# tsurumeso/vocal-remover

Hardware: AMD Instinct MI355X
Metric: spectrogram-frames/sec (inference, CascadedNet n_fft=2048) (higher is better)
Workload: dtype f32; 1 GPU; configs[1]: 30 s stereo 44.1 kHz synthetic song, STFT -> 11 crops of 256 frames in one device batch -> predict_mask -> stitch -> mask apply -> iSTFT x2; n_fft=2048, hop=1024, cropsize=256, parallelism=replicas x1 (songs shard, no collective), input_residency=inputs resident in HBM when the timed region starts

## Files before the change

### vocal-remover_amd/csrc/conv_x3h.hip

```cpp
#include <cstdlib>
#include <type_traits>

#include "conv_epilogue.h"
#include "conv_stage.h"
#include "kernels.h"
#include "lds_dma.h"
#include "x3h_common.h"

namespace vr {

template <int MT, int TH, bool UP = true>
struct X3hCfg {
    static constexpr int TW = 32, CK = 8, KK = 9;
    static constexpr int TH_in = TH + 2, PW = TW + 2;
    static constexpr int NSLOT = TH_in * PW;
    static constexpr int NPASS = (NSLOT + 255) / 256;
    static constexpr int WM = MT / 32, WN = TH / 4;
    static constexpr int PLANE = NSLOT * 16;
    static constexpr int P_BYTES = 2 * PLANE;
    static constexpr int NWP = KK * 2 * MT;
    static constexpr int W_BYTES = NWP * 16;
    static constexpr int NWPASS = (NWP + 255) / 256;
    static constexpr int LROWS = TH / 2 + 3, LW = 20, LSLOT = LROWS * LW;
    static constexpr int L_OFF = P_BYTES + 2 * W_BYTES;
    static constexpr int L_BYTES = UP ? CK * LSLOT * 4 : 0;
    static constexpr int E_OFF = L_OFF + L_BYTES;
    static constexpr int M_OFF = E_OFF + 4 * MT * 4;
    static constexpr int LDS_BYTES = M_OFF + 16;
    static constexpr int OCC = (MT == 32 && TH == 8) ? 3 : 2;
    static constexpr int NXL = 8 * NPASS, NWMIN = (NWP / 64) / 4;
    static constexpr int NG = 14;
    static_assert(TH % 4 == 0 && MT % 32 == 0 && LDS_BYTES <= 80 * 1024 && 2 * NXL + NWMIN < 64 && NXL <= 30 && LSLOT <= 256, "tile");
};

__device__ long long g_x3h_trace[4 * 4 * 6 * 8];
void x3h_trace_read(long long* host, int n) {
    VR_HIP(hipMemcpyFromSymbol(host, HIP_SYMBOL(g_x3h_trace), sizeof(long long) * (size_t)(n < 768 ? n : 768)));
}
void x3h_trace_clear() {
    static long long zeros[768] = {0};
    VR_HIP(hipMemcpyToSymbol(HIP_SYMBOL(g_x3h_trace), zeros, sizeof zeros));
}

template <int MT, int TH, bool UP, bool HI, bool TRACE = false>
__global__ __launch_bounds__(256, (X3hCfg<MT, TH>::OCC + (HI ? 1 : 0))) void conv_x3h_kernel(const ConvArgs a) {
    using Cfg = X3hCfg<MT, TH, UP>;
    constexpr int TW = Cfg::TW, KK = Cfg::KK, PW = Cfg::PW, NSLOT = Cfg::NSLOT, NPASS = Cfg::NPASS, WM = Cfg::WM, WN = Cfg::WN,
                  PLANE = Cfg::PLANE, NWP = Cfg::NWP, NWPASS = Cfg::NWPASS;
    extern __shared__ __attribute__((aligned(16))) char smem_x3h[];
    char* const Pb = smem_x3h;

    const int id = blockIdx.x;
    const int xcd = id & 7;
    const int rr = id >> 3;
    const int ct = rr % a.nct;
    const int per_xcd = (a.npt + 7) >> 3;
    const int pt = (a.dbg & 16) ? (rr / a.nct) * 8 + xcd : xcd * per_xcd + rr / a.nct;
    if (pt >= a.npt) return;
    const int tiles_per_img = a.tiles_h * a.tiles_w;
    const int n = pt / tiles_per_img;
    const int trem = pt - n * tiles_per_img;
    const int h0 = (trem / a.tiles_w) * TH;
    const int w0 = (a.wt0 + trem % a.tiles_w) * TW;
    const int co0 = ct * MT;
    const int tid = threadIdx.x;
    const int lane = tid & 63;
    const int wave = __builtin_amdgcn_readfirstlane(tid >> 6);
    const int nchunk = (a.Cin + 7) >> 3;
    const unsigned lds0 = (unsigned)(size_t)smem_x3h;
    const int dbg = a.dbg & 15;
    const bool prio = (a.dbg & 32) != 0;
    const int trace_wg = TRACE ? (int)blockIdx.x - (int)(gridDim.x / 2) : -1;
    auto stamp = [&](int k, int point) {
        if (TRACE && trace_wg >= 0 && trace_wg < 4 && k >= 2 && k < 8) {
            const long long t = __builtin_readcyclecounter();
            if (lane == 0) g_x3h_trace[((trace_wg * 4 + wave) * 6 + (k - 2)) * 8 + point] = t;
        }
    };

    auto pixel_offset = [&](int p, unsigned sH4) -> int {
        const int s = p * 256 + tid;
        const int r = s / PW, c = s - r * PW;
        const int hi = h0 - 1 + r, wi = w0 - 1 + c;
        const bool ok = s < NSLOT && hi >= 0 && hi < a.Hin && wi >= 0 && wi < a.Win;
        return ok ? (int)((unsigned)hi * sH4 + (unsigned)(wi * 4)) : (int)0x80000000u;
    };
    const ConvSrc& us = a.src[0].up ? a.src[0] : (a.src[1].up ? a.src[1] : a.src[2]);
    constexpr bool any_up = UP;
    int lrow = 0, lcol4 = 0;
    int lidx[NPASS], lstep[NPASS];
    float lh[NPASS], lw_[NPASS];
// ... 8 lines not shown
            const int s = p * 256 + tid;
            const int r = s / PW, c = s - r * PW;
            const int hi = h0 - 1 + r, wi = w0 - 1 + c;
            const bool ok = s < NSLOT && hi >= 0 && hi < a.Hin && wi >= 0 && wi < a.Win;
            const float h1r = us.rh * (float)(ok ? hi : 0), w1r = us.rw * (float)(ok ? wi : 0);
            const int h1 = (int)h1r, w1 = (int)w1r;
            lidx[p] = ok ? ((h1 - lr0) * Cfg::LW + (w1 - lc0)) * 32 : -1;
            const int rs = (h1 + 1 < us.H && h1 + 1 - lr0 < Cfg::LROWS) ? Cfg::LW * 32 : 0;
            const int cs = (w1 + 1 < us.W && w1 + 1 - lc0 < Cfg::LW) ? 32 : 0;
            lstep[p] = (rs << 16) | cs;
            lh[p] = h1r - (float)h1;
            lw_[p] = w1r - (float)w1;
        }
    }
    unsigned woff0;
    {
        const int q = wave * 64 + lane;
        const int m = q % MT, tp = q / MT;
        woff0 = (unsigned)((tp * a.CoutPad + m) * 16);
    }
    const unsigned wstep = (unsigned)((256 / MT) * a.CoutPad * 16);
    const long long wchunk_bytes = (long long)KK * 2 * a.CoutPad * 16;
    auto issue_w = [&](int k) {
        const char* wb = static_cast<const char*>(a.x3w) + k * wchunk_bytes + (long long)co0 * 16;
        const i32x4 wr = make_rsrc(reinterpret_cast<const float*>(wb), (unsigned)(wchunk_bytes - (long long)co0 * 16));
        const unsigned ws_b = lds0 + (unsigned)(Cfg::P_BYTES + (k & 1) * Cfg::W_BYTES);
#pragma unroll
        for (int i = 0; i < NWPASS; ++i) {
            const int pp = wave + 4 * i;
            if ((pp + 1) * 64 <= NWP) dma16s(ws_b + pp * 1024, woff0, wr, (unsigned)i * wstep);
            else if (pp * 64 + lane < NWP) dma16s(ws_b + pp * 1024, woff0, wr, (unsigned)i * wstep);
        }
    };
    const float* xp = a.src[0].p + (long long)n * a.src[0].sN;
    long long xsC = a.src[0].sC;
    unsigned xsH4 = (unsigned)a.src[0].sH * 4u;
    int xend = a.c1, xsi = 0;
    bool xup = a.src[0].up != 0;
    unsigned upm[2] = {0u, 0u};
    int xvo[NPASS];
#pragma unroll
    for (int p = 0; p < NPASS; ++p) xvo[p] = pixel_offset(p, xsH4);
    auto next_source = [&]() {
        ++xsi;
        if (xsi == 1) { xp = a.src[1].p + (long long)n * a.src[1].sN; xsC = a.src[1].sC; xsH4 = (unsigned)a.src[1].sH * 4u; xend = a.c2; xup = a.src[1].up != 0; }
        else { xp = a.src[2].p + (long long)n * a.src[2].sN; xsC = a.src[2].sC; xsH4 = (unsigned)a.src[2].sH * 4u; xend = 1 << 30; xup = a.src[2].up != 0; }
#pragma unroll
        for (int p = 0; p < NPASS; ++p) xvo[p] = pixel_offset(p, xsH4);
    };
    float xr[2][NPASS][8];
    auto load_channel = [&](int k, int cl, auto par) {
        constexpr int PAR = decltype(par)::value;
        const int ci = k * 8 + cl;
        const bool live = ci < a.Cin && dbg != 1;
        if (live && ci >= xend) next_source();
        if (live && ci >= xend) next_source();
        const i32x4 xs = make_rsrc(xp, live ? 0x7FFFFFF0u : 0u);
        const bool up = UP && live && xup;
        if (cl == 0) upm[PAR] = 0u;
        upm[PAR] |= (up ? 1u : 0u) << cl;
        xr[PAR][0][cl] = x3h_load(xs, up ? (int)((unsigned)lrow * xsH4) + lcol4 : xvo[0]);
        const i32x4 xs1 = make_rsrc(xp, (live && !up) ? 0x7FFFFFF0u : 0u);
#pragma unroll
        for (int p = 1; p < NPASS; ++p) xr[PAR][p][cl] = x3h_load(xs1, xvo[p]);
        if (live) xp += xsC;
    };
    auto wait_pixels = [&](auto par, auto newer) {
        constexpr int PAR = decltype(par)::value, NEWER = decltype(newer)::value;
#pragma unroll
        for (int p = 0; p < NPASS; ++p) x3h_wait8<NEWER>(xr[PAR][p]);
    };
    auto stage_lowres = [&](auto par) {
        constexpr int PAR = decltype(par)::value;
        if (upm[PAR] == 0u) return;
        if (tid < Cfg::LSLOT) {
            vr_f32x4h lo4, hi4;
// ... 79 lines not shown
    };

    const int khalf = lane >> 5, l31 = lane & 31;
    const int bq = (wave * WN * PW + l31) * 16;
    const int bX = bq + khalf * PLANE, bY1 = bq + khalf * 16, bY2 = bq + khalf * (PW - 2) * 16;
    const int aX = l31 * 16, aY = (MT + l31 + khalf * 2 * MT) * 16;

    f32x16 acc[WM][WN];
#pragma unroll
    for (int mi = 0; mi < WM; ++mi)
#pragma unroll
        for (int ni = 0; ni < WN; ++ni)
#pragma unroll
            for (int r = 0; r < 16; ++r) acc[mi][ni][r] = 0.f;

    using P0 = std::integral_constant<int, 0>;
    using P1 = std::integral_constant<int, 1>;
    float ecv[4];
    {
        const int ec = co0 + (tid & (MT - 1));
        const int ecc = ec < a.Cout ? ec : a.Cout - 1;
        const i32x4 rb = make_rsrc(a.bias, a.bias ? 0x7FFFFFF0u : 0u);
        const i32x4 re = make_rsrc(a.epi, a.epi ? 0x7FFFFFF0u : 0u);
        const i32x4 rw = make_rsrc(reinterpret_cast<const float*>(static_cast<const char*>(a.x3w) + nchunk * wchunk_bytes), 0x7FFFFFF0u);
        ecv[0] = x3h_load(rb, ecc * 4);
        ecv[1] = x3h_load(re, ecc * 8);
        ecv[2] = x3h_load(re, ecc * 8 + 4);
        ecv[3] = x3h_load(rw, ec * 4);
    }
    auto follow = [&](int e, bool first) {
        const int need = 140 - (e < 14 ? 14 : e);
        shlo = (first || need < shlo) ? need : shlo;
        int nsh = sh;
        if (first || need < sh - 1) nsh = need;
        else if (need > sh + 12) {
            nsh = need < sh + 64 ? need : sh + 64;
            nsh = nsh < shlo + 64 ? nsh : shlo + 64;
            nsh = nsh > sh ? nsh : sh;
        }
        if (nsh != sh) {
            if (!first) {
                const int d = nsh - sh;
                const float f = d < -126 ? 0.f : x3h_pow2(d);
#pragma unroll
                for (int mi = 0; mi < WM; ++mi)
#pragma unroll
                    for (int ni = 0; ni < WN; ++ni)
#pragma unroll
                        for (int r = 0; r < 16; ++r) acc[mi][ni][r] *= f;
            }
            sh = nsh;
            psc = x3h_pow2(sh);
        }
    };
#pragma unroll
    for (int cl = 0; cl < 8; ++cl) load_channel(0, cl, P0{});
    issue_w(0);
#pragma unroll
    for (int cl = 0; cl < 8; ++cl) load_channel(1, cl, P1{});
    wait_pixels(P0{}, std::integral_constant<int, Cfg::NXL + Cfg::NWMIN>{});
    asm volatile("; landed %0 %1 %2 %3" : "+v"(ecv[0]), "+v"(ecv[1]), "+v"(ecv[2]), "+v"(ecv[3]));
    if (tid < MT) {
        float* E = reinterpret_cast<float*>(smem_x3h + Cfg::E_OFF);
        E[tid] = ecv[0];
        E[MT + tid] = a.epi ? ecv[1] : 1.f;
        E[2 * MT + tid] = a.epi ? ecv[2] : 0.f;
        E[3 * MT + tid] = ecv[3];
    }
    post_max(P0{});
    if (any_up) stage_lowres(P0{});
    lds_barrier();
    follow(read_max_exp(), true);
    convert(P0{});
    asm volatile("s_waitcnt vmcnt(%0) lgkmcnt(0)" :: "n"(Cfg::NXL) : "memory");
    __builtin_amdgcn_s_barrier();
    asm volatile("" ::: "memory");

    auto chunk = [&](int k, auto par) {
        constexpr int PAR = decltype(par)::value;
        const bool more = k + 1 < nchunk;
        stamp(k, 0);
        {
            const char* Wb = smem_x3h + Cfg::P_BYTES + PAR * Cfg::W_BYTES;
            vr_f16x8 A[2][WM], B[2][WN];
            auto read_group = [&](int g, int buf) {
                const bool isY = g == 13 || (g < 12 && g % 3 == 2);
                const int t = g >= 12 ? 8 : 2 * (g / 3) + (g % 3 == 1 ? 1 : 0);
                const int ty = t / 3, tx = t % 3;
#pragma unroll
                for (int mi = 0; mi < WM; ++mi) {
                    const char* q = Wb + (t * 2 * MT + mi * 32) * 16;
                    if (!isY) A[buf][mi] = *reinterpret_cast<const vr_f16x8*>(q + aX);
                    else if (t < 8) A[buf][mi] = *reinterpret_cast<const vr_f16x8*>(q + aY);
                    else {
                        const vr_i32x4 v = *reinterpret_cast<const vr_i32x4*>(q + aX + MT * 16);
                        vr_i32x4 z;
#pragma unroll
                        for (int j = 0; j < 4; ++j) z[j] = khalf ? 0 : v[j];
                        A[buf][mi] = __builtin_bit_cast(vr_f16x8, z);
// ... 18 lines not shown
            if (prio) __builtin_amdgcn_s_setprio(1);
#pragma unroll
            for (int g = 0; g < Cfg::NG; ++g) {
                const int cur = g & 1;
                if (g + 1 < Cfg::NG) read_group(g + 1, cur ^ 1);
                if (more) {
                    if (g == 0) issue_w(k + 1);
                    if (g >= 1 && g <= 4) { load_channel(k + 2, 2 * g - 2, par); load_channel(k + 2, 2 * g - 1, par); }
                }
                __builtin_amdgcn_sched_barrier(0);
                mfma_group(cur);
                __builtin_amdgcn_sched_barrier(0);
            }
            if (prio) __builtin_amdgcn_s_setprio(0);
        }
        stamp(k, 1);
        if (more) {
            using Q = std::integral_constant<int, PAR ^ 1>;
            wait_pixels(Q{}, std::integral_constant<int, Cfg::NXL + Cfg::NWMIN>{});
            stamp(k, 2);
            post_max(Q{});
            if (any_up) stage_lowres(Q{});
            stamp(k, 3);
            lds_barrier();
            stamp(k, 4);
            follow(read_max_exp(), false);
            if (dbg != 3) convert(Q{});
            stamp(k, 5);
            asm volatile("s_waitcnt vmcnt(%0) lgkmcnt(0)" :: "n"(Cfg::NXL) : "memory");
            stamp(k, 6);
            __builtin_amdgcn_s_barrier();
            asm volatile("" ::: "memory");
            stamp(k, 7);
        }
    };
    for (int k = 0; k < nchunk; k += 2) {
        chunk(k, P0{});
        if (k + 1 < nchunk) chunk(k + 1, P1{});
    }
    asm volatile("s_waitcnt vmcnt(0)" ::: "memory");

    if (dbg == 4) return;
    {
        const float fo = x3h_pow2(-sh);
        const float* Wi = reinterpret_cast<const float*>(smem_x3h + Cfg::E_OFF) + 3 * MT;
#pragma unroll
        for (int mi = 0; mi < WM; ++mi)
#pragma unroll
            for (int rq = 0; rq < 4; ++rq) {
                const vr_f32x4h wi = *reinterpret_cast<const vr_f32x4h*>(Wi + mi * 32 + 8 * rq + 4 * khalf);
#pragma unroll
                for (int ni = 0; ni < WN; ++ni)
#pragma unroll
                    for (int j = 0; j < 4; ++j) acc[mi][ni][rq * 4 + j] = (acc[mi][ni][rq * 4 + j] * fo) * wi[j];
            }
    }
    {
        int hon[WN], won[WN];
#pragma unroll
        for (int ni = 0; ni < WN; ++ni) { hon[ni] = h0 + wave * WN + ni; won[ni] = w0 + l31; }
        epi_store<MT, WM, WN>(VR_EPI_ARGS(a), acc, reinterpret_cast<const float*>(smem_x3h + Cfg::E_OFF), n, co0, khalf,
                              h0 + TH <= a.Hout && w0 + TW <= a.Wout, hon, won);
    }
    if (a.part) {
        __syncthreads();
        float* red = reinterpret_cast<float*>(smem_x3h);
#pragma unroll
        for (int mi = 0; mi < WM; ++mi) {
#pragma unroll
            for (int r = 0; r < 16; ++r) {
                float s1 = 0.f, s2 = 0.f;
#pragma unroll
                for (int ni = 0; ni < WN; ++ni) {
                    const int ho = h0 + wave * WN + ni, wo = w0 + l31;
                    if (ho < a.Hout && wo < a.Wout) {
                        const float v = acc[mi][ni][r];
                        s1 += v;
                        s2 = fmaf(v, v, s2);
                    }
                }
                s1 = half_wave_sum_dpp(s1);
                s2 = half_wave_sum_dpp(s2);
                if (l31 == 16) {
                    const int m = mi * 32 + (r & 3) + 8 * (r >> 2) + 4 * khalf;
                    red[(wave * MT + m) * 2 + 0] = s1;
                    red[(wave * MT + m) * 2 + 1] = s2;
                }
// ... 60 lines not shown
}
__global__ void x3h_wscale_batched_kernel(const X3WDesc* __restrict__ d) {
    const X3WDesc e = d[blockIdx.y];
    x3h_wscale_block(e.w, e.o, e.Cin, e.KK, e.CoutPad, blockIdx.x);
}
__global__ void x3h_weights_batched_kernel(const X3WDesc* __restrict__ d) {
    const X3WDesc e = d[blockIdx.y];
    x3h_weights_elem(e.w, e.o, e.Cin, e.KK, e.CoutPad, (long long)blockIdx.x * blockDim.x + threadIdx.x);
}

void launch_x3h_weights(const float* w, void* o, int Cin, int KK, int CoutPad, hipStream_t st) {
    const long long n = (long long)((Cin + 7) / 8 * 8) * KK * CoutPad;
    VR_LAUNCH(x3h_wscale_kernel, dim3((unsigned)((CoutPad + 31) / 32)), dim3(256), 0, st, w, o, Cin, KK, CoutPad);
    VR_LAUNCH(x3h_weights_kernel, dim3((unsigned)((n + 255) / 256)), dim3(256), 0, st, w, o, Cin, KK, CoutPad);
    VR_HIP(hipGetLastError());
}
void launch_x3h_weights_batched(const X3WDesc* d_descs, int n, long long max_elems, int max_cout_pad, hipStream_t st) {
    if (n <= 0) return;
    VR_LAUNCH(x3h_wscale_batched_kernel, dim3((unsigned)((max_cout_pad + 31) / 32), (unsigned)n), dim3(256), 0, st, d_descs);
    VR_LAUNCH(x3h_weights_batched_kernel, dim3((unsigned)((max_elems + 255) / 256), (unsigned)n), dim3(256), 0, st, d_descs);
    VR_HIP(hipGetLastError());
}

template <int MT, int TH, bool UP, bool HI, bool TRACE = false>
static void x3h_launch_up(const ConvArgs& a, hipStream_t st) {
    using Cfg = X3hCfg<MT, TH, UP>;
    auto kern = conv_x3h_kernel<MT, TH, UP, HI, TRACE>;
    static std::atomic<unsigned long long> attr_done{0};
    ensure_lds_attr(attr_done, reinterpret_cast<const void*>(kern), Cfg::LDS_BYTES);
    const int groups = (a.npt + 7) / 8;
    VR_LAUNCH(kern, dim3(groups * 8 * a.nct), dim3(256), Cfg::LDS_BYTES, st, a);
    VR_HIP(hipGetLastError());
}

template <int MT, int TH>
static void x3h_launch(const ConvArgs& a, hipStream_t st) {
    static const int hi = [] { const char* e = getenv("VR_X3H_HI"); return e ? atoi(e) : 0; }();
    if (a.dbg & 64) {
        if (a.src[0].up | a.src[1].up | a.src[2].up) x3h_launch_up<MT, TH, true, false, true>(a, st);
        else x3h_launch_up<MT, TH, false, false, true>(a, st);
        return;
    }
    if (a.src[0].up | a.src[1].up | a.src[2].up) x3h_launch_up<MT, TH, true, false>(a, st);
    else if (hi && TH == 8) x3h_launch_up<MT, TH, false, (TH == 8)>(a, st);
    else x3h_launch_up<MT, TH, false, false>(a, st);
}

void x3h_launch_conv(const ConvArgs& a, const X3Tile& t, hipStream_t st) {
    if (t.MT == 64) x3h_launch<64, 8>(a, st);
    else if (t.TH == 16) x3h_launch<32, 16>(a, st);
    else x3h_launch<32, 8>(a, st);
}

}
```

### vocal-remover_amd/csrc/model.h

```cpp
#pragma once
#include <chrono>
#include <deque>
#include <functional>
#include <map>
#include <memory>
#include <string>
#include <vector>

#include "kernels.h"

namespace vr {

struct Arena {
    char* base = nullptr;
    size_t cap = 0, off = 0, peak = 0;
    bool dry = false;
    void* alloc(size_t bytes) {
        const size_t a = (off + 255) & ~size_t(255);
        off = a + bytes;
        if (off > peak) peak = off;
        if (dry) return reinterpret_cast<void*>(uintptr_t(256));
        if (off > cap) throw Error(-4, "workspace arena overflow (planning bug)");
        return base + a;
    }
// ... 166 lines not shown
    bool band_fork_active = false;
    bool gs_clear_pending = false;
    bool wgrad_on_side = false;
    struct Lane { hipStream_t main = nullptr, side = nullptr; hipEvent_t fork = nullptr, join = nullptr, start = nullptr, done = nullptr; Arena ws; };
    std::vector<Lane> lanes;
    void swap_lane(int i);

private:
    float* p_arena = nullptr; size_t p_floats = 0;
    float* b_arena = nullptr; size_t b_floats = 0;
    Arena ws;
    Arena io;
    void ensure_ws(size_t bytes);
    int plan_B = -1, plan_T = -1; bool plan_training = false; size_t plan_peak = 0;
    void ensure_io(size_t bytes);

    std::deque<BN> bns;
    std::vector<BN*> bn_list;
    std::vector<Conv*> wino_list;
    struct PendingConv { ConvArgs a; ConvShape shp; double flops, bytes; bool stats; BNFinalizeArgs fin; BN* bn; };
    std::vector<PendingConv>* conv_sink = nullptr;
    int x3d_mode = 2;
    int conv_w_lo = 0, conv_w_hi = 0;
    std::vector<Conv*> x3d_list;
    float* wino_arena = nullptr;
    float* winot_arena = nullptr;
    std::map<const Param*, float*> winot_of;
    char* wino6_arena = nullptr;
    char* winot6_arena = nullptr;
    std::map<const Param*, void*> winot6_of;
    char* x3_arena = nullptr;
    char* x3t_arena = nullptr;
    std::map<const Param*, void*> x3t_of;
    std::map<const Param*, void*> x3dt_of;
    std::vector<WgReduceDesc> wred_host, wred_sent;
    WgReduceDesc* wred_dev = nullptr;
    size_t wred_cap = 0;
    void flush_wgrad_sums();
    struct X3Batch { std::vector<X3WDesc> host; X3WDesc* dev = nullptr; long long max_elems = 0; };
    X3Batch xb_fwd, xb_bwd;
    void run_x3_batch(X3Batch& b, std::vector<X3WDesc>& descs);
    void refresh_wino(bool with_dgrad);
    struct WinoBatch { std::vector<WinoWDesc> host; WinoWDesc* dev = nullptr; long long max_elems = 0; };
    WinoBatch wb_fwd, wb_bwd, wb_fwd6, wb_bwd6;
    void run_wino_batch(WinoBatch& b, std::vector<WinoWDesc>& descs, bool split6);
    BNFoldDesc* d_fold = nullptr;
// ... 119 lines not shown
```

### vocal-remover_amd/csrc/model.hip

```cpp
#include "model.h"

#include <algorithm>
#include <chrono>
#include <cmath>
#include <cstdlib>
#include <cstring>

namespace vr {

static inline int round_up(int v, int m) { return (v + m - 1) / m * m; }

Param* Model::add_param(const std::string& key, std::vector<int64_t> shape, ParamKind kind, bool trainable) {
    params.emplace_back();
    Param* p = &params.back();
    p->key = key;
    p->shape = std::move(shape);
    p->kind = kind;
    p->trainable = trainable;
    p->numel = 1;
    for (auto d : p->shape) p->numel *= (size_t)d;
    p->dev_numel = p->numel;
    if (kind == PK_CONV) {
        p->Cout = (int)p->shape[0];
        p->Cin = (int)p->shape[1];
// ... 77 lines not shown
    ihr->Cout = 4 * hid; ihr->Cin = nin_lstm; ihr->KK = 1; ihr->CoutPad = M.proj.CoutPad; ihr->co_off = 4 * hid;
    ihr->dev_numel = 0; ihr->alias_of = ihf;
    M.proj.w = ihf;
    M.dense.name = q + ".dense";
    M.dense.Cin = 2 * hid; M.dense.Cout = nin_lstm; M.dense.CoutPad = round_up(nin_lstm, 32);
    M.dense.KS = 1; M.dense.stride = 1; M.dense.pad_h = M.dense.pad_w = 0; M.dense.slope = 0.f;
    M.dense.w = add_param(q + ".dense.0.weight", {nin_lstm, 2 * hid}, PK_CONV, true);
    M.dense_b = add_param(q + ".dense.0.bias", {nin_lstm}, PK_PLAIN, true);
    M.dense.bn = add_bn(q + ".dense.1", nin_lstm, 0);
    build_cba(B.dec[3], p + ".dec1.conv1", 3 * c + 1, c, 3, 1, 1, 1, 1, 1, RELU);
}

Model::Model(int device_, int n_fft_, int hop_, int nout_, int nout_lstm_, bool is_complex_)
    : device(device_), n_fft(n_fft_), hop(hop_), nout(nout_), nout_lstm(nout_lstm_), is_complex(is_complex_), nin(is_complex_ ? 4 : 2) {
    VR_CHECK(n_fft >= 64 && (n_fft & (n_fft - 1)) == 0 && n_fft <= 8192, -2, "n_fft must be a power of two in [64, 8192]");
    VR_CHECK(hop > 0, -2, "hop_length must be positive");
    VR_CHECK(nout % 4 == 0 && nout >= 4 && nout_lstm % 4 == 0 && nout_lstm >= 4, -2, "nout / nout_lstm must be multiples of 4");
    max_bin = n_fft / 2;
    output_bin = n_fft / 2 + 1;
    VR_CHECK((max_bin / 2) % 16 == 0, -2, "n_fft/4 must be a multiple of 16 (four stride-2 encoders)");
    DeviceGuard dev_guard(device);
    if (const char* e = getenv("VR_MFMA_MODE")) { mfma_mode = atoi(e); VR_CHECK(mfma_mode >= 0 && mfma_mode <= 3, -2, "VR_MFMA_MODE: 0, 1, 2 or 3"); }
    default_mfma_mode = mfma_mode;
    VR_HIP(hipStreamCreateWithFlags(&stream, hipStreamNonBlocking));
    if (!getenv("VR_NO_SIDE_STREAM")) {
        VR_HIP(hipStreamCreateWithFlags(&side_stream, hipStreamNonBlocking));
        VR_HIP(hipEventCreateWithFlags(&ev_fork, hipEventDisableTiming));
        VR_HIP(hipEventCreateWithFlags(&ev_join, hipEventDisableTiming));
        if (!getenv("VR_NO_SPLIT_BATCH")) {
            int k = getenv("VR_LANES") ? atoi(getenv("VR_LANES")) : 2;
            k = k < 1 ? 1 : (k > 4 ? 4 : k);
            lanes.resize(k - 1);
            for (Lane& l : lanes) {
                VR_HIP(hipStreamCreateWithFlags(&l.main, hipStreamNonBlocking));
                VR_HIP(hipStreamCreateWithFlags(&l.side, hipStreamNonBlocking));
                VR_HIP(hipEventCreateWithFlags(&l.fork, hipEventDisableTiming));
                VR_HIP(hipEventCreateWithFlags(&l.join, hipEventDisableTiming));
                VR_HIP(hipEventCreateWithFlags(&l.start, hipEventDisableTiming));
                VR_HIP(hipEventCreateWithFlags(&l.done, hipEventDisableTiming));
            }
        }
    }
    const int nin_lstm = max_bin / 2;
    build_basenet(nets_[0], "stg1_low_band_net.0", nin, nout / 2, nin_lstm / 2, nout_lstm);
    build_cba(tail1, "stg1_low_band_net.1", nout / 2, nout / 4, 1, 1, 0, 0, 1, 1, 0.f);
    build_basenet(nets_[1], "stg1_high_band_net", nin, nout / 4, nin_lstm / 2, nout_lstm / 2);
// ... 186 lines not shown
        const int G = 4 * M.hid;
        if (!M.bias_sum) VR_HIP(hipMalloc(reinterpret_cast<void**>(&M.bias_sum), (size_t)2 * G * sizeof(float)));
        launch_add(M.b_ih_f->dev, M.b_hh_f->dev, M.bias_sum, G, stream);
        launch_add(M.b_ih_r->dev, M.b_hh_r->dev, M.bias_sum + G, G, stream);
    }
    affine_dirty = false;
}

void Model::set_option(const std::string& name, int value) {
    plan_peak = 0;
    if (name == "train_winograd") train_wino = value != 0;
    else if (name == "serial_exec") serial = value != 0;
    else if (name == "params_dirty") affine_dirty = true;
    else if (name == "mfma_bf16") { mfma_mode = value != 0 ? 1 : default_mfma_mode; affine_dirty = true; }
    else if (name == "mfma_mode") {
        if (value < -1 || value > 3) throw Error(-2, "mfma_mode: 0, 1, 2, 3 or -1 (default)");
        mfma_mode = value < 0 ? default_mfma_mode : value; affine_dirty = true;
    }
    else if (name == "conv_x3d") {
        if (value < -1 || value > 2) throw Error(-2, "conv_x3d: 0, 1, 2 or -1 (default)");
        x3d_mode = value < 0 ? 2 : value;
    }
    else if (name == "crop_window") crop_window = value != 0;
    else if (name == "adam_reset") reset_adam_state();
    else if (name == "hip_graph" || name == "conv_x3p" || name == "wgrad_x3h" || name == "conv_x3b") {
        static std::string told;
        if (told.find("|" + name + "|") == std::string::npos) {
            told += "|" + name + "|";
            fprintf(stderr, "libvr_mi355: option '%s' was retired with its kernel (tools/experiments/README.md); ignored\n", name.c_str());
        }
    }
    else throw Error(-2, "unknown option: " + name);
}

void Model::refresh_wino(bool with_dgrad) {
    if (!wino_arena) {
        size_t total = 0;
        for (Conv* L : wino_list) total += (size_t)L->Cin * 16 * L->CoutPad;
        VR_HIP(hipMalloc(reinterpret_cast<void**>(&wino_arena), total * sizeof(float)));
        size_t off = 0;
        for (Conv* L : wino_list) { L->wino = wino_arena + off; off += (size_t)L->Cin * 16 * L->CoutPad; }
    }
    {
        std::vector<WinoWDesc> d;
        for (Conv* L : wino_list) d.push_back(WinoWDesc{L->w->dev, L->wino, L->Cin, L->CoutPad});
        run_wino_batch(wb_fwd, d, false);
// ... 349 lines not shown
            if (!x3_pick(probe, ConvShape{L.KS, L.stride, L.dh, L.dw}, &xt)) {
                for (SrcSpec& sp : srcs) {
                    if (!sp.up) continue;
                    const Tensor& t = sp.t;
                    Tensor u;
                    u.N = t.N; u.C = t.C; u.H = 2 * t.H; u.W = 2 * t.W;
                    u.sH = u.W; u.sC = (long long)u.H * u.W; u.sN = u.sC * u.C; u.slope = 1.f;
                    u.p = ws.allocf((size_t)u.N * u.C * u.H * u.W);
                    if (!dry) launch_upsample2x(t, u.p, stream);
                    sp = SrcSpec{u};
                }
                build_fwd_args(L, srcs, N, batch_as_h, a);
            }
        }
    }
    a.bias = bias;
    const bool fuse_epi = !training && L.bn != nullptr;
    if (fuse_epi) { a.epi = L.bn->affine; a.epi_slope = L.slope; }
    a.wino = (training && !train_wino) ? nullptr : L.wino;
    a.wino6 = (a.wino && mfma_mode == 2) ? L.wino6 : nullptr;
    a.x3w = (x3_mode() && !(training && !train_wino)) ? L.x3w : nullptr;
    if (!x3d_mode && a.Win == 16) a.x3w = nullptr;
    a.bf16 = mfma_mode;
    int wcols = a.Wout;
    if (conv_w_hi > 0 && !training && mfma_mode == 3 && !batch_as_h && !conv_sink) {
        X3Tile xt;
        int tth;
        const ConvShape cs{L.KS, L.stride, L.dh, L.dw};
        if (!thin16_pick(a, cs, &tth) && x3_pick(a, cs, &xt)) {
            a.w_lo = conv_w_lo; a.w_hi = conv_w_hi;
            wcols = std::min(a.Wout, (conv_w_hi + 31) / 32 * 32) - conv_w_lo / 32 * 32;
        }
    }
    Tensor o;
    if (batch_as_h) {
        o.N = N; o.C = L.Cout; o.H = 1; o.W = a.Wout;
        if (out_view) { o.p = out_view->p; o.g = out_view->g; o.sN = out_view->sN; o.sC = out_view->sC; o.sH = out_view->sH; }
        else {
            o.p = ws.allocf((size_t)N * L.Cout * a.Wout); o.sN = (long long)L.Cout * a.Wout; o.sC = a.Wout; o.sH = a.Wout;
            if (taping()) o.g = galloc((size_t)N * L.Cout * a.Wout, false);
        }
        a.dst[0] = ConvDst{o.p, 0, o.sC, o.sN, 0};
    } else {
        o.N = N; o.C = L.Cout; o.H = a.Hout; o.W = a.Wout;
        if (out_view) {
            VR_CHECK(out_view->H == a.Hout && out_view->W == a.Wout && out_view->C == L.Cout, -2, "conv " + L.name + ": output view shape mismatch");
// ... 1483 lines not shown
        for (Part& p : parts) {
            VR_CHECK(p.o.out_off == p.need, -4, "stream schedule mismatch (planning bug)");
            if (!out_on_dev && p.need > 0) {
                VR_HIP(hipMemcpy2DAsync(y[p.k], (size_t)capacity[p.k] * 4, p.stage_y, (size_t)p.need * 4, (size_t)p.need * 4, 2, hipMemcpyDeviceToHost, stream));
                VR_HIP(hipMemcpy2DAsync(v[p.k], (size_t)capacity[p.k] * 4, p.stage_v, (size_t)p.need * 4, (size_t)p.need * 4, 2, hipMemcpyDeviceToHost, stream));
            }
        }
        VR_HIP(hipStreamSynchronize(stream));
    } catch (...) {
        hipStreamSynchronize(stream);
        throw;
    }
    for (Part& p : parts) {
        p.S->broken = false;
        if (n_out) n_out[p.k] = p.need;
    }
}

void Model::debug_conv(const float* x, int N, int Cin, int H, int W, const float* w_oihw, int Cout, int KS, int stride,
                       int dh, int dw, int flags, const float* aff, float slope, const float* bias, float* out,
                       float* stats_out) {
    DeviceGuard dev_guard(device);
    const int up = flags & 1;
    const bool want_wino = (flags & 2) != 0, epi = (flags & 4) != 0;
    const int KK = KS * KS, CoutPad = round_up(Cout, 32);
    const int Hin = up ? 2 * H : H, Win = up ? 2 * W : W;
    const int pad_h = KS == 1 ? 0 : dh, pad_w = KS == 1 ? 0 : dw;
    const int Hout = (Hin + 2 * pad_h - dh * (KS - 1) - 1) / stride + 1;
    const int Wout = (Win + 2 * pad_w - dw * (KS - 1) - 1) / stride + 1;
    std::vector<float> wk((size_t)Cin * KK * CoutPad, 0.f);
    for (int co = 0; co < Cout; ++co)
        for (int ci = 0; ci < Cin; ++ci)
            for (int k = 0; k < KK; ++k) wk[((size_t)ci * KK + k) * CoutPad + co] = w_oihw[((size_t)co * Cin + ci) * KK + k];
    float *dx, *dw_, *dout, *daff = nullptr, *dbias = nullptr, *dpart = nullptr;
    const size_t xin = (size_t)N * Cin * H * W, xout = (size_t)N * Cout * Hout * Wout;
    VR_HIP(hipMalloc(&dx, xin * 4)); VR_HIP(hipMalloc(&dw_, wk.size() * 4)); VR_HIP(hipMalloc(&dout, xout * 4));
    VR_HIP(hipMemcpy(dx, x, xin * 4, hipMemcpyHostToDevice));
    VR_HIP(hipMemcpy(dw_, wk.data(), wk.size() * 4, hipMemcpyHostToDevice));
    const size_t naff = epi ? Cout : Cin;
    if (aff) { VR_HIP(hipMalloc(&daff, naff * 8)); VR_HIP(hipMemcpy(daff, aff, naff * 8, hipMemcpyHostToDevice)); }
    if (bias) { VR_HIP(hipMalloc(&dbias, (size_t)Cout * 4)); VR_HIP(hipMemcpy(dbias, bias, (size_t)Cout * 4, hipMemcpyHostToDevice)); }
    Tensor t;
    t.p = dx; t.N = N; t.C = Cin; t.H = H; t.W = W; t.sH = W; t.sC = (long long)H * W; t.sN = t.sC * Cin;
    if (!epi) { t.aff0 = daff; t.slope = slope; }
    ConvArgs a{};
    a.nsrc = 1; a.src[0] = make_src(t, up != 0, 0); a.c1 = a.c2 = Cin; a.Cin = Cin;
    a.w = dw_; a.bias = dbias; a.Cout = Cout; a.CoutPad = CoutPad;
    if (epi && daff) { a.epi = daff; a.epi_slope = slope; }
    a.bf16 = mfma_mode;
    float* dwino = nullptr;
    void* dwino6 = nullptr;
    void* dx3w = nullptr;
    if (want_wino && mfma_mode == 3 && stride == 1 && (KS == 1 || dh > 1)) {
        VR_HIP(hipMalloc(&dx3w, x3_weights_bytes(Cin, KK, CoutPad)));
        launch_x3h_weights(dw_, dx3w, Cin, KK, CoutPad, stream);
        a.x3w = dx3w;
    } else if (want_wino) {
        VR_CHECK(KS == 3 && stride == 1 && dh == 1 && dw == 1, -2, "Winograd weights exist for 3x3 stride-1 convs only");
        VR_HIP(hipMalloc(&dwino, (size_t)Cin * 16 * CoutPad * 4));
        launch_wino_weights(dw_, dwino, Cin, CoutPad, stream);
        a.wino = dwino;
        if (mfma_mode == 2) {
            VR_HIP(hipMalloc(&dwino6, wino_weights6_bytes(Cin, CoutPad)));
            launch_wino_weights6(dw_, dwino6, Cin, CoutPad, stream);
            a.wino6 = dwino6;
            VR_HIP(hipMalloc(&dx3w, x3_weights_bytes(Cin, 9, CoutPad)));
            launch_x3_weights(dw_, dx3w, Cin, 9, CoutPad, stream);
            a.x3w = dx3w;
        }
// ... 2 lines not shown
            launch_x3h_weights(dw_, dx3w, Cin, 9, CoutPad, stream);
            a.x3w = dx3w;
        }
    }
    if (!x3d_mode && Win == 16) a.x3w = nullptr;
    a.dst[0] = ConvDst{dout, (long long)Hout * Wout * Cout, (long long)Hout * Wout, (long long)Wout, 0};
    a.d1 = a.d2 = 1 << 30;
    a.N = N; a.Hout = Hout; a.Wout = Wout; a.Hin = Hin; a.Win = Win; a.pad_h = pad_h; a.pad_w = pad_w;
    const ConvShape shp{KS, stride, dh, dw};
    size_t npt = 0;
    if (stats_out) { npt = conv_part_count(a, shp); VR_HIP(hipMalloc(&dpart, npt * Cout * 8)); a.part = dpart; }
    launch_conv(a, shp, stream);
    VR_HIP(hipStreamSynchronize(stream));
    VR_HIP(hipMemcpy(out, dout, xout * 4, hipMemcpyDeviceToHost));
    if (stats_out) {
        std::vector<float> part(npt * Cout * 2);
        VR_HIP(hipMemcpy(part.data(), dpart, part.size() * 4, hipMemcpyDeviceToHost));
        for (int c = 0; c < Cout; ++c) {
            double s1 = 0, s2 = 0;
            for (size_t i = 0; i < npt; ++i) { s1 += part[(i * Cout + c) * 2]; s2 += part[(i * Cout + c) * 2 + 1]; }
            stats_out[2 * c] = (float)s1; stats_out[2 * c + 1] = (float)s2;
        }
    }
    hipFree(dx); hipFree(dw_); hipFree(dout); hipFree(daff); hipFree(dbias); hipFree(dpart); hipFree(dwino); hipFree(dwino6); hipFree(dx3w);
}

}
```

### vocal-remover_amd/csrc/vr_common.h

```cpp
#pragma once
#include <hip/hip_runtime.h>
#include <atomic>
#include <cstdint>
#include <cstdio>
#include <stdexcept>
#include <string>
#include <vector>

namespace vr {

struct Error : std::runtime_error {
    int code;
    Error(int c, const std::string& m) : std::runtime_error(m), code(c) {}
};

#define VR_HIP(expr)                                                                              \
    do {                                                                                          \
        hipError_t _e = (expr);                                                                   \
        if (_e != hipSuccess)                                                                     \
            throw ::vr::Error(-3, std::string(#expr) + ": " + hipGetErrorString(_e));             \
    } while (0)

#define VR_CHECK(cond, code, msg)                                                                 \
    do {                                                                                          \
// ... 81 lines not shown
    int nsrc, c1, c2;
    int Cin;
    const float* w;
    const float* wino;
    const void* wino6;
    const void* x3w;
    const float* bias;
    int Cout, CoutPad;
    ConvDst dst[3];
    int d1, d2;
    float* part;
    const float* epi;
    float epi_slope;
    int N, Hout, Wout, Hin, Win;
    int pad_h, pad_w;
    int tiles_w, tiles_h, npt, nct;
    int dbg;
    int bf16;
    long long s2_cls_stride;
    int s2_H, s2_W;
    int tapmask;
    int w_lo, w_hi;
    int wt0;
};

struct ConvShape {
    int KS, stride, dil_h, dil_w;
};

struct WgradArgs {
    ConvArgs in;
    const float* dz;
    long long zN, zC, zH;
    int Cout, CoutPad;
    float* part;
    long long part_stride;
    int P, tiles_w, tiles_h, npt, nchunks, nct;
    int dma;
    int bf16;
    int allow_wino;
};
double launch_wgrad(const WgradArgs& a, const ConvShape& s, float* grad_out, int accumulate, hipStream_t st);
struct WgReduceDesc { const float* part; long long stride; float* out; long long n; int P; int accumulate; long long blk0; };
void wgrad_defer_to(std::vector<WgReduceDesc>* sink);
int wgrad_reduce_vec(const WgReduceDesc* host_descs, int n);
void launch_wgrad_reduce_batched(const WgReduceDesc* d_descs, int n, long long total_blocks, int vec, hipStream_t st);
// ... 9 lines not shown
```

Baseline: 173,900 spectrogram-frames/sec.

## Split input-channel reduction across two wave groups in 3x3 conv kernel

Adds a K-split variant of the 32x8 x3h conv kernel. It launches 512 threads, and two 256-thread groups each take alternate 8-channel chunks. The groups sync through an LDS atomic spin barrier, align their shared exponent scale, and reduce partial accumulators through LDS before one group runs the epilogue. The variant is picked during inference when there are many channel chunks but fewer than roughly one workgroup per CU, so that small-grid layers can use more waves. The cost is double the LDS per workgroup, the spin-barrier overhead and an extra reduction pass.

```diff
diff --git a/vocal-remover_amd/csrc/conv_x3h.hip b/vocal-remover_amd/csrc/conv_x3h.hip
--- a/vocal-remover_amd/csrc/conv_x3h.hip
+++ b/vocal-remover_amd/csrc/conv_x3h.hip
@@ -28,6 +28,8 @@
     static constexpr int M_OFF = E_OFF + 4 * MT * 4;
     static constexpr int LDS_BYTES = M_OFF + 16;
     static constexpr int OCC = (MT == 32 && TH == 8) ? 3 : 2;
+    static constexpr int KS_STRIDE = LDS_BYTES + 16;
+    static constexpr int KS_LDS_BYTES = 2 * KS_STRIDE;
     static constexpr int NXL = 8 * NPASS, NWMIN = (NWP / 64) / 4;
     static constexpr int NG = 14;
     static_assert(TH % 4 == 0 && MT % 32 == 0 && LDS_BYTES <= 80 * 1024 && 2 * NXL + NWMIN < 64 && NXL <= 30 && LSLOT <= 256, "tile");
@@ -42,12 +44,26 @@
     VR_HIP(hipMemcpyToSymbol(HIP_SYMBOL(g_x3h_trace), zeros, sizeof zeros));
 }
 
-template <int MT, int TH, bool UP, bool HI, bool TRACE = false>
-__global__ __launch_bounds__(256, (X3hCfg<MT, TH>::OCC + (HI ? 1 : 0))) void conv_x3h_kernel(const ConvArgs a) {
+__device__ __forceinline__ void x3h_group_barrier(int* cnt, int target, int lane) {
+    asm volatile("" ::: "memory");
+    if (lane == 0) __hip_atomic_fetch_add(cnt, 1, __ATOMIC_RELAXED, __HIP_MEMORY_SCOPE_WORKGROUP);
+    for (int spin = 0; spin < (1 << 22); ++spin) {
+        const int v = __builtin_amdgcn_readfirstlane(__hip_atomic_load(cnt, __ATOMIC_RELAXED, __HIP_MEMORY_SCOPE_WORKGROUP));
+        if (v >= target) break;
+        __builtin_amdgcn_s_sleep(1);
+    }
+    asm volatile("" ::: "memory");
+}
+
+template <int MT, int TH, bool UP, bool HI, bool TRACE = false, bool KS = false>
+__global__ __launch_bounds__(KS ? 512 : 256, (X3hCfg<MT, TH>::OCC + (HI ? 1 : 0))) void conv_x3h_kernel(const ConvArgs a) {
     using Cfg = X3hCfg<MT, TH, UP>;
+    static_assert(!KS || (MT == 32 && TH == 8 && !UP && HI && !TRACE), "the K-split form exists for the plain 32 x 8 tiling only");
     constexpr int TW = Cfg::TW, KK = Cfg::KK, PW = Cfg::PW, NSLOT = Cfg::NSLOT, NPASS = Cfg::NPASS, WM = Cfg::WM, WN = Cfg::WN,
                   PLANE = Cfg::PLANE, NWP = Cfg::NWP, NWPASS = Cfg::NWPASS;
-    extern __shared__ __attribute__((aligned(16))) char smem_x3h[];
+    extern __shared__ __attribute__((aligned(16))) char smem_x3h_wg[];
+    const int grp = KS ? __builtin_amdgcn_readfirstlane((int)threadIdx.x >> 8) : 0;
+    char* const smem_x3h = smem_x3h_wg + (KS ? grp * Cfg::KS_STRIDE : 0);
     char* const Pb = smem_x3h;
 
     const int id = blockIdx.x;
@@ -63,10 +79,12 @@
     const int h0 = (trem / a.tiles_w) * TH;
     const int w0 = (a.wt0 + trem % a.tiles_w) * TW;
     const int co0 = ct * MT;
-    const int tid = threadIdx.x;
+    const int tid = KS ? (int)(threadIdx.x & 255) : (int)threadIdx.x;
     const int lane = tid & 63;
     const int wave = __builtin_amdgcn_readfirstlane(tid >> 6);
-    const int nchunk = (a.Cin + 7) >> 3;
+    const int nchunk_all = (a.Cin + 7) >> 3;
+    const int nchunk = KS ? (nchunk_all - grp + 1) >> 1 : nchunk_all;
+    auto gch = [&](int j) -> int { return KS ? 2 * j + grp : j; };
     const unsigned lds0 = (unsigned)(size_t)smem_x3h;
     const int dbg = a.dbg & 15;
     const bool prio = (a.dbg & 32) != 0;
@@ -121,7 +139,7 @@
     const unsigned wstep = (unsigned)((256 / MT) * a.CoutPad * 16);
     const long long wchunk_bytes = (long long)KK * 2 * a.CoutPad * 16;
     auto issue_w = [&](int k) {
-        const char* wb = static_cast<const char*>(a.x3w) + k * wchunk_bytes + (long long)co0 * 16;
+        const char* wb = static_cast<const char*>(a.x3w) + gch(k) * wchunk_bytes + (long long)co0 * 16;
         const i32x4 wr = make_rsrc(reinterpret_cast<const float*>(wb), (unsigned)(wchunk_bytes - (long long)co0 * 16));
         const unsigned ws_b = lds0 + (unsigned)(Cfg::P_BYTES + (k & 1) * Cfg::W_BYTES);
 #pragma unroll
@@ -150,7 +168,19 @@
     float xr[2][NPASS][8];
     auto load_channel = [&](int k, int cl, auto par) {
         constexpr int PAR = decltype(par)::value;
-        const int ci = k * 8 + cl;
+        const int ci = gch(k) * 8 + cl;
+        if constexpr (KS) {
+            if (cl == 0 && gch(k) > 0) {
+#pragma unroll
+                for (int c = 0; c < 8; ++c) {
+                    const int cs = ci - 8 + c;
+                    const bool lv = cs < a.Cin && dbg != 1;
+                    if (lv && cs >= xend) next_source();
+                    if (lv && cs >= xend) next_source();
+                    if (lv) xp += xsC;
+                }
+            }
+        }
         const bool live = ci < a.Cin && dbg != 1;
         if (live && ci >= xend) next_source();
         if (live && ci >= xend) next_source();
@@ -276,7 +306,7 @@
         const int ecc = ec < a.Cout ? ec : a.Cout - 1;
         const i32x4 rb = make_rsrc(a.bias, a.bias ? 0x7FFFFFF0u : 0u);
         const i32x4 re = make_rsrc(a.epi, a.epi ? 0x7FFFFFF0u : 0u);
-        const i32x4 rw = make_rsrc(reinterpret_cast<const float*>(static_cast<const char*>(a.x3w) + nchunk * wchunk_bytes), 0x7FFFFFF0u);
+        const i32x4 rw = make_rsrc(reinterpret_cast<const float*>(static_cast<const char*>(a.x3w) + nchunk_all * wchunk_bytes), 0x7FFFFFF0u);
         ecv[0] = x3h_load(rb, ecc * 4);
         ecv[1] = x3h_load(re, ecc * 8);
         ecv[2] = x3h_load(re, ecc * 8 + 4);
@@ -307,28 +337,44 @@
             psc = x3h_pow2(sh);
         }
     };
-#pragma unroll
-    for (int cl = 0; cl < 8; ++cl) load_channel(0, cl, P0{});
-    issue_w(0);
-#pragma unroll
-    for (int cl = 0; cl < 8; ++cl) load_channel(1, cl, P1{});
-    wait_pixels(P0{}, std::integral_constant<int, Cfg::NXL + Cfg::NWMIN>{});
-    asm volatile("; landed %0 %1 %2 %3" : "+v"(ecv[0]), "+v"(ecv[1]), "+v"(ecv[2]), "+v"(ecv[3]));
-    if (tid < MT) {
-        float* E = reinterpret_cast<float*>(smem_x3h + Cfg::E_OFF);
-        E[tid] = ecv[0];
-        E[MT + tid] = a.epi ? ecv[1] : 1.f;
-        E[2 * MT + tid] = a.epi ? ecv[2] : 0.f;
-        E[3 * MT + tid] = ecv[3];
-    }
-    post_max(P0{});
-    if (any_up) stage_lowres(P0{});
-    lds_barrier();
-    follow(read_max_exp(), true);
-    convert(P0{});
-    asm volatile("s_waitcnt vmcnt(%0) lgkmcnt(0)" :: "n"(Cfg::NXL) : "memory");
-    __builtin_amdgcn_s_barrier();
-    asm volatile("" ::: "memory");
+    int* const gcnt = reinterpret_cast<int*>(smem_x3h + Cfg::LDS_BYTES);
+    int gbar = 0;
+    auto sync_waves = [&]() {
+        if constexpr (KS) { gbar += 4; x3h_group_barrier(gcnt, gbar, lane); }
+        else __builtin_amdgcn_s_barrier();
+    };
+    auto sync_lds = [&]() {
+        if constexpr (KS) { asm volatile("s_waitcnt lgkmcnt(0)" ::: "memory"); sync_waves(); }
+        else lds_barrier();
+    };
+    if constexpr (KS) {
+        if (tid == 0) *gcnt = 0;
+        lds_barrier();
+    }
+    if (!KS || nchunk > 0) {
+#pragma unroll
+        for (int cl = 0; cl < 8; ++cl) load_channel(0, cl, P0{});
+        issue_w(0);
+#pragma unroll
+        for (int cl = 0; cl < 8; ++cl) load_channel(1, cl, P1{});
+        wait_pixels(P0{}, std::integral_constant<int, Cfg::NXL + Cfg::NWMIN>{});
+        asm volatile("; landed %0 %1 %2 %3" : "+v"(ecv[0]), "+v"(ecv[1]), "+v"(ecv[2]), "+v"(ecv[3]));
+        if (tid < MT) {
+            float* E = reinterpret_cast<float*>(smem_x3h + Cfg::E_OFF);
+            E[tid] = ecv[0];
+            E[MT + tid] = a.epi ? ecv[1] : 1.f;
+            E[2 * MT + tid] = a.epi ? ecv[2] : 0.f;
+            E[3 * MT + tid] = ecv[3];
+        }
+        post_max(P0{});
+        if (any_up) stage_lowres(P0{});
+        sync_lds();
+        follow(read_max_exp(), true);
+        convert(P0{});
+        asm volatile("s_waitcnt vmcnt(%0) lgkmcnt(0)" :: "n"(Cfg::NXL) : "memory");
+        sync_waves();
+        asm volatile("" ::: "memory");
+    }
 
     auto chunk = [&](int k, auto par) {
         constexpr int PAR = decltype(par)::value;
@@ -393,14 +439,14 @@
             post_max(Q{});
             if (any_up) stage_lowres(Q{});
             stamp(k, 3);
-            lds_barrier();
+            sync_lds();
             stamp(k, 4);
             follow(read_max_exp(), false);
             if (dbg != 3) convert(Q{});
             stamp(k, 5);
             asm volatile("s_waitcnt vmcnt(%0) lgkmcnt(0)" :: "n"(Cfg::NXL) : "memory");
             stamp(k, 6);
-            __builtin_amdgcn_s_barrier();
+            sync_waves();
             asm volatile("" ::: "memory");
             stamp(k, 7);
         }
@@ -411,6 +457,47 @@
     }
     asm volatile("s_waitcnt vmcnt(0)" ::: "memory");
 
+    if constexpr (KS) {
+        constexpr int NO_SH = 1 << 20;
+        int* const shp = reinterpret_cast<int*>(smem_x3h + Cfg::M_OFF);
+        if (tid == 0) *shp = nchunk > 0 ? sh : NO_SH;
+        lds_barrier();
+        const int sh0 = *reinterpret_cast<const int*>(smem_x3h_wg + Cfg::M_OFF);
+        const int sh1 = *reinterpret_cast<const int*>(smem_x3h_wg + Cfg::KS_STRIDE + Cfg::M_OFF);
+        const int shj = __builtin_amdgcn_readfirstlane(sh0 < sh1 ? sh0 : sh1);
+        const int d = shj - (nchunk > 0 ? sh : NO_SH);
+        if (d != 0) {
+            const float f = d < -126 ? 0.f : x3h_pow2(d);
+#pragma unroll
+            for (int ni = 0; ni < WN; ++ni)
+#pragma unroll
+                for (int r = 0; r < 16; ++r) acc[0][ni][r] *= f;
+        }
+        sh = shj;
+        static_assert(3 * 8192 <= Cfg::KS_STRIDE && 8192 <= Cfg::E_OFF && WM == 1 && WN == 2, "hand-over buffers");
+        char* const xq = (wave < 3 ? smem_x3h_wg + Cfg::KS_STRIDE + wave * 8192 : smem_x3h_wg) + lane * 16;
+        if (grp == 1) {
+#pragma unroll
+            for (int ni = 0; ni < WN; ++ni)
+#pragma unroll
+                for (int rq = 0; rq < 4; ++rq) {
+                    vr_f32x4h v;
+#pragma unroll
+                    for (int j = 0; j < 4; ++j) v[j] = acc[0][ni][rq * 4 + j];
+                    *reinterpret_cast<vr_f32x4h*>(xq + (ni * 4 + rq) * 1024) = v;
+                }
+        }
+        lds_barrier();
+        if (grp == 1) return;
+#pragma unroll
+        for (int ni = 0; ni < WN; ++ni)
+#pragma unroll
+            for (int rq = 0; rq < 4; ++rq) {
+                const vr_f32x4h v = *reinterpret_cast<const vr_f32x4h*>(xq + (ni * 4 + rq) * 1024);
+#pragma unroll
+                for (int j = 0; j < 4; ++j) acc[0][ni][rq * 4 + j] += v[j];
+            }
+    }
     if (dbg == 4) return;
     {
         const float fo = x3h_pow2(-sh);
@@ -433,7 +520,7 @@
         epi_store<MT, WM, WN>(VR_EPI_ARGS(a), acc, reinterpret_cast<const float*>(smem_x3h + Cfg::E_OFF), n, co0, khalf,
                               h0 + TH <= a.Hout && w0 + TW <= a.Wout, hon, won);
     }
-    if (a.part) {
+    if (!KS && a.part) {
         __syncthreads();
         float* red = reinterpret_cast<float*>(smem_x3h);
 #pragma unroll
@@ -540,15 +627,25 @@
     VR_HIP(hipGetLastError());
 }
 
-template <int MT, int TH, bool UP, bool HI, bool TRACE = false>
+template <int MT, int TH, bool UP, bool HI, bool TRACE = false, bool KS = false>
 static void x3h_launch_up(const ConvArgs& a, hipStream_t st) {
     using Cfg = X3hCfg<MT, TH, UP>;
-    auto kern = conv_x3h_kernel<MT, TH, UP, HI, TRACE>;
+    auto kern = conv_x3h_kernel<MT, TH, UP, HI, TRACE, KS>;
+    constexpr int lds = KS ? Cfg::KS_LDS_BYTES : Cfg::LDS_BYTES;
     static std::atomic<unsigned long long> attr_done{0};
-    ensure_lds_attr(attr_done, reinterpret_cast<const void*>(kern), Cfg::LDS_BYTES);
+    ensure_lds_attr(attr_done, reinterpret_cast<const void*>(kern), lds);
     const int groups = (a.npt + 7) / 8;
-    VR_LAUNCH(kern, dim3(groups * 8 * a.nct), dim3(256), Cfg::LDS_BYTES, st, a);
+    VR_LAUNCH(kern, dim3(groups * 8 * a.nct), dim3(KS ? 512 : 256), lds, st, a);
     VR_HIP(hipGetLastError());
+}
+
+constexpr double X3H_KS_MAX_WG_PER_CU = 1.0;
+constexpr int X3H_KS_MIN_CHUNKS = 10;
+static bool x3h_ksplit_pick(const ConvArgs& a) {
+    if (a.ksplit <= 0 || a.part || (a.dbg & 64) || (a.src[0].up | a.src[1].up | a.src[2].up)) return false;
+    if (a.ksplit >= 2) return true;
+    const long long wgs = (long long)((a.npt + 7) / 8) * 8 * a.nct;
+    return (a.Cin + 7) / 8 >= X3H_KS_MIN_CHUNKS && (double)wgs < X3H_KS_MAX_WG_PER_CU * 256.0;
 }
 
 template <int MT, int TH>
@@ -560,6 +657,7 @@
         return;
     }
     if (a.src[0].up | a.src[1].up | a.src[2].up) x3h_launch_up<MT, TH, true, false>(a, st);
+    else if (MT == 32 && TH == 8 && x3h_ksplit_pick(a)) x3h_launch_up<32, 8, false, true, false, true>(a, st);
     else if (hi && TH == 8) x3h_launch_up<MT, TH, false, (TH == 8)>(a, st);
     else x3h_launch_up<MT, TH, false, false>(a, st);
 }
diff --git a/vocal-remover_amd/csrc/model.h b/vocal-remover_amd/csrc/model.h
--- a/vocal-remover_amd/csrc/model.h
+++ b/vocal-remover_amd/csrc/model.h
@@ -212,6 +212,7 @@
     std::vector<PendingConv>* conv_sink = nullptr;
     int x3d_mode = 2;
     int conv_w_lo = 0, conv_w_hi = 0;
+    int x3h_ksplit = 1, default_x3h_ksplit = 1;
     std::vector<Conv*> x3d_list;
     float* wino_arena = nullptr;
     float* winot_arena = nullptr;
diff --git a/vocal-remover_amd/csrc/model.hip b/vocal-remover_amd/csrc/model.hip
--- a/vocal-remover_amd/csrc/model.hip
+++ b/vocal-remover_amd/csrc/model.hip
@@ -123,6 +123,8 @@
     DeviceGuard dev_guard(device);
     if (const char* e = getenv("VR_MFMA_MODE")) { mfma_mode = atoi(e); VR_CHECK(mfma_mode >= 0 && mfma_mode <= 3, -2, "VR_MFMA_MODE: 0, 1, 2 or 3"); }
     default_mfma_mode = mfma_mode;
+    if (const char* e = getenv("VR_X3H_KSPLIT")) { x3h_ksplit = atoi(e); VR_CHECK(x3h_ksplit >= 0 && x3h_ksplit <= 2, -2, "VR_X3H_KSPLIT: 0, 1 or 2"); }
+    default_x3h_ksplit = x3h_ksplit;
     VR_HIP(hipStreamCreateWithFlags(&stream, hipStreamNonBlocking));
     if (!getenv("VR_NO_SIDE_STREAM")) {
         VR_HIP(hipStreamCreateWithFlags(&side_stream, hipStreamNonBlocking));
@@ -355,6 +357,10 @@
         x3d_mode = value < 0 ? 2 : value;
     }
     else if (name == "crop_window") crop_window = value != 0;
+    else if (name == "x3h_ksplit") {
+        if (value < -1 || value > 2) throw Error(-2, "x3h_ksplit: 0, 1, 2 or -1 (default)");
+        x3h_ksplit = value < 0 ? default_x3h_ksplit : value;
+    }
     else if (name == "adam_reset") reset_adam_state();
     else if (name == "hip_graph" || name == "conv_x3p" || name == "wgrad_x3h" || name == "conv_x3b") {
         static std::string told;
@@ -750,6 +756,7 @@
     a.x3w = (x3_mode() && !(training && !train_wino)) ? L.x3w : nullptr;
     if (!x3d_mode && a.Win == 16) a.x3w = nullptr;
     a.bf16 = mfma_mode;
+    a.ksplit = training ? 0 : x3h_ksplit;
     int wcols = a.Wout;
     if (conv_w_hi > 0 && !training && mfma_mode == 3 && !batch_as_h && !conv_sink) {
         X3Tile xt;
@@ -2279,6 +2286,9 @@
                        float* stats_out) {
     DeviceGuard dev_guard(device);
     const int up = flags & 1;
+    const int csplit = flags >> 8;
+    VR_CHECK(csplit >= 0 && csplit < Cin && !(csplit && up), -2, "vr_debug_conv2d: the concat split must lie inside the channels (no upsample)");
+    VR_CHECK(!((flags & 8) && stats_out), -2, "vr_debug_conv2d: an eval launch has no BatchNorm statistics");
     const bool want_wino = (flags & 2) != 0, epi = (flags & 4) != 0;
     const int KK = KS * KS, CoutPad = round_up(Cout, 32);
     const int Hin = up ? 2 * H : H, Win = up ? 2 * W : W;
@@ -2302,6 +2312,18 @@
     if (!epi) { t.aff0 = daff; t.slope = slope; }
     ConvArgs a{};
     a.nsrc = 1; a.src[0] = make_src(t, up != 0, 0); a.c1 = a.c2 = Cin; a.Cin = Cin;
+    float* dx2 = nullptr;
+    if (csplit) {
+        const size_t c2n = (size_t)(Cin - csplit) * H * W + W;
+        VR_HIP(hipMalloc(&dx2, (size_t)N * c2n * 4));
+        for (int n = 0; n < N; ++n)
+            VR_HIP(hipMemcpy(dx2 + n * c2n, x + ((size_t)n * Cin + csplit) * H * W, (size_t)(Cin - csplit) * H * W * 4, hipMemcpyHostToDevice));
+        Tensor t2 = t;
+        t2.p = dx2; t2.C = Cin - csplit; t2.sN = (long long)c2n;
+        a.src[0].C = csplit;
+        a.nsrc = 2; a.src[1] = make_src(t2, false, 0); a.c1 = csplit;
+    }
+    if (flags & 8) a.ksplit = x3h_ksplit;
     a.w = dw_; a.bias = dbias; a.Cout = Cout; a.CoutPad = CoutPad;
     if (epi && daff) { a.epi = daff; a.epi_slope = slope; }
     a.bf16 = mfma_mode;
@@ -2350,7 +2372,7 @@
             stats_out[2 * c] = (float)s1; stats_out[2 * c + 1] = (float)s2;
         }
     }
-    hipFree(dx); hipFree(dw_); hipFree(dout); hipFree(daff); hipFree(dbias); hipFree(dpart); hipFree(dwino); hipFree(dwino6); hipFree(dx3w);
-}
-
-}
+    hipFree(dx); hipFree(dw_); hipFree(dout); hipFree(daff); hipFree(dbias); hipFree(dpart); hipFree(dwino); hipFree(dwino6); hipFree(dx3w); hipFree(dx2);
+}
+
+}
diff --git a/vocal-remover_amd/csrc/vr_common.h b/vocal-remover_amd/csrc/vr_common.h
--- a/vocal-remover_amd/csrc/vr_common.h
+++ b/vocal-remover_amd/csrc/vr_common.h
@@ -127,6 +127,7 @@
     int tapmask;
     int w_lo, w_hi;
     int wt0;
+    int ksplit;
 };
 
 struct ConvShape {
```

Result: no change. 173,600 spectrogram-frames/sec (median of 4 runs) (-0.1%).
